# Arktis2022/Spiking-Diffusion

Measured on AMD Instinct MI355X. Metric: images/sec + LIF-kernel HBM GB/s, MNIST 100-step sample T=16, 1->8 GPU, higher is better.
Workload: dtype fp32-exact (4 fp6 digits x fp4 spikes on the block-scaled MFMA + certified decisions + exact 6-digit recomputation of flagged neurons)

## Files before the change

### spiking-diffusion_amd/csrc/cert_common.h

```cpp
#pragma once
#include "den_common.h"
#include <math.h>

typedef int v6i __attribute__((ext_vector_type(6)));
typedef int v8i __attribute__((ext_vector_type(8)));
typedef float v2f __attribute__((ext_vector_type(2)));
typedef float v16f __attribute__((ext_vector_type(16)));

constexpr int T16 = 16;
constexpr int POSB = 256;
constexpr int WT = 64 * 24;
constexpr float CERT_4EPS = 4.0f * 2.38418579e-07f;

constexpr unsigned FLAG_CAP = 1u << 20;
static inline long long spk_cert_bitmap_words(long long n) { return (n + 31) / 32; }
static inline long long spk_cert_ticket_idx(long long n) { return 2 + (long long)FLAG_CAP + spk_cert_bitmap_words(n); }
static inline long long spk_cert_flag_words(long long n) { return spk_cert_ticket_idx(n) + 1; }
struct CertWs { unsigned* flags; unsigned flag_cap; long long ticket_idx; };
static inline CertWs spk_cert_ws(unsigned* flag_words, int flag_cap, long long n) {
  return CertWs{flag_words, flag_cap < 0 || (unsigned)flag_cap > FLAG_CAP ? FLAG_CAP : (unsigned)flag_cap, spk_cert_ticket_idx(n)};
}

__device__ __forceinline__ unsigned* spk_cert_bitmap(const CertWs& ws) { return ws.flags + 2 + FLAG_CAP; }

__device__ __forceinline__ void spk_cert_flag(const CertWs& ws, long long n, bool flagged = true) {
  if (flagged) {
    const unsigned idx = atomicAdd(ws.flags, 1u);
    if (idx < ws.flag_cap) ws.flags[2 + idx] = (unsigned)n;
    else atomicOr(spk_cert_bitmap(ws) + (n >> 5), 1u << (n & 31));
  }
}

__device__ __forceinline__ void spk_cert_handover(const CertWs& ws) {
  if (atomicAdd(ws.flags + ws.ticket_idx, 1u) == gridDim.x - 1) {
    ws.flags[1] = atomicAdd(ws.flags, 0u);
    ws.flags[0] = 0u;
    ws.flags[ws.ticket_idx] = 0u;
  }
}

template <bool WG, class I, class Fix>
__device__ __forceinline__ void spk_cert_scan(const CertWs& ws, unsigned count, I unit, I n_units, long long n_words, bool clearer,
                                              Fix&& fix) {
  const unsigned nlist = count < ws.flag_cap ? count : ws.flag_cap;
  for (I e = unit; e < nlist; e += n_units) fix((long long)ws.flags[2 + e]);
  if (count > ws.flag_cap) {
    unsigned* bm = spk_cert_bitmap(ws);
    long long w0 = unit, w1 = n_words, step = n_units;
    if (WG) {
      const long long per = (n_words + n_units - 1) / n_units;
      w0 = (long long)unit * per;
      w1 = w0 + per < n_words ? w0 + per : n_words;
      step = 1;
    }
    for (long long wi = w0; wi < w1; wi += step) {
      unsigned wd = bm[wi];
      if (WG) __syncthreads();
      if (wd && clearer) bm[wi] = 0u;
      while (wd) {
        const int bit = __ffs((int)wd) - 1;
        wd &= wd - 1;
        fix(wi * 32 + bit);
      }
    }
  }
}

__device__ __forceinline__ void spk_cert_add_active8(long long& part, unsigned nib, const int4& q0, const int4& q1) {
  part += (nib & 0x0000000fu) ? (long long)q0.x : 0ll;
  part += (nib & 0x000000f0u) ? (long long)q0.y : 0ll;
  part += (nib & 0x00000f00u) ? (long long)q0.z : 0ll;
  part += (nib & 0x0000f000u) ? (long long)q0.w : 0ll;
  part += (nib & 0x000f0000u) ? (long long)q1.x : 0ll;
  part += (nib & 0x00f00000u) ? (long long)q1.y : 0ll;
  part += (nib & 0x0f000000u) ? (long long)q1.z : 0ll;
  part += (nib & 0xf0000000u) ? (long long)q1.w : 0ll;
}
__device__ __forceinline__ long long spk_join64(int lo, int hi) {
  return (long long)(((unsigned long long)(unsigned)hi << 32) | (unsigned)lo);
}
__device__ __forceinline__ long long spk_shfl64(long long v, int src) {
  return spk_join64(__shfl((int)(unsigned)(v & 0xffffffffll), src), __shfl((int)(v >> 32), src));
}
__device__ __forceinline__ long long spk_cert_sum_quarters(long long part) {
#pragma unroll
  for (int off = 16; off <= 32; off <<= 1)
    part += spk_join64(__shfl_xor((int)(unsigned)(part & 0xffffffffll), off), __shfl_xor((int)(part >> 32), off));
  return part;
}
__device__ __forceinline__ float exact_preact(double s, double sc, double bi) { return (float)fma(s, sc, bi); }
__device__ __forceinline__ void spk_cert_patch_nibble(uint8_t* rec, int co, bool spike) {
  const int byte = (co & 31) >> 1;
  unsigned* wp = reinterpret_cast<unsigned*>(rec + (byte & ~3));
  const unsigned shw = 8u * (byte & 3) + 4u * (co & 1);
  atomicAnd(wp, ~(0xFu << shw));
  if (spike) atomicOr(wp, 0x2u << shw);
}

__device__ __forceinline__ double spk_cert_quantise(float w, int sh) { return rint(ldexp((double)w, sh)); }
__device__ __forceinline__ void spk_cert_scale_bias(double* scale, double* bias_d, const float* bias, int co, int sh) {
  scale[co] = ldexp(1.0, -sh);
  bias_d[co] = bias ? (double)bias[co] : 0.0;
}
template <class Q>
__device__ __forceinline__ void spk_cert_emit_fragment(uint8_t* tile, int ln, int digit, bool live, Q&& q) {
  unsigned bits[6] = {0, 0, 0, 0, 0, 0};
  for (int k = 0; k < 32 && live; ++k) {
    int dg[6];
    spk_balanced_digits<5>(q(k), dg);
    int d = 0;
#pragma unroll
    for (int p = 0; p < 6; ++p) d = (p == digit) ? dg[p] : d;
    const unsigned code = spk_e2m3_code(d);
    const int bit = 6 * k, wd = bit >> 5, sft = bit & 31;
#pragma unroll
    for (int q2 = 0; q2 < 6; ++q2) {
      if (q2 == wd) bits[q2] |= code << sft;
      if (q2 == wd + 1 && sft > 26) bits[q2] |= code >> (32 - sft);
    }
  }
  unsigned* d16 = reinterpret_cast<unsigned*>(tile + ln * 16);
  unsigned* d8 = reinterpret_cast<unsigned*>(tile + 1024 + ln * 8);
  d16[0] = bits[0]; d16[1] = bits[1]; d16[2] = bits[2]; d16[3] = bits[3];
  d8[0] = bits[4]; d8[1] = bits[5];
}
```

### spiking-diffusion_amd/csrc/den_mfma_fp6v2.hip

```cpp
#include "cert_common.h"
#include "../../include/spkdiff.h"
#include <stdlib.h>
#include <type_traits>
#include <utility>

namespace {

constexpr int CK = 32;
constexpr int N_PAIR = 18;
constexpr int N_D4 = 5;
constexpr int N_MAIN = N_PAIR + N_D4;
constexpr int N_L5 = 2;
constexpr int NACC = 2;
constexpr int W_PIECES = (N_PAIR * WT + 1023) / 1024;
constexpr int W_LDS = W_PIECES * 1024;
constexpr int W_SLAB = ((N_MAIN + N_L5) * WT + 1023) / 1024 * 1024;

struct V2Args {
  const uint8_t* in0; int nch;
  const uint8_t* wq; const double* scale; const double* bias; const float* wl1;
  const float* bn_a; const float* bn_b;
  uint8_t* out; uint8_t* out_cnt;
  CertWs ws;
  int handover;
// ... 606 lines not shown
#pragma unroll
        for (int r = 0; r < 16; ++r) {
          const int rowA = spk_acc_row(r, 0);
          const int c0 = __builtin_amdgcn_readlane(cnt[i], rowA), c1 = __builtin_amdgcn_readlane(cnt[i], rowA + 4);
          cntv[r] = half ? c1 : c0;
        }
      }
      int nmax_rec = 0;
      if constexpr (REC) nmax_rec = s_nmax[BSKIP ? p_out[i] : 2 * (wave + NWV * i) + half];
      float zmax = 0.f, dmin = 3.0e38f;
      int nmax = nmax_rec;
#pragma unroll
      for (int r2 = 0; r2 < 16; r2 += 2) {
        const v2f p0 = {acc[i][0][r2], acc[i][0][r2 + 1]}, p1 = {acc[i][1][r2], acc[i][1][r2 + 1]};
        const v2f q4 = __builtin_elementwise_fma(p0, (v2f){1024.0f, 1024.0f}, p1);
        const v2f z2 = __builtin_elementwise_fma(q4, (v2f){Ac4, Ac4}, (v2f){Bc, Bc});
        if constexpr (!REC) nmax = max(nmax, max(cntv[r2], cntv[r2 + 1]));
#pragma unroll
        for (int e = 0; e < 2; ++e) {
          const float z = z2[e];
          zmax = fmaxf(zmax, fabsf(z));
          const float h = fmaf(z - v, 0.5f, v);
          const float hm = h - 1.0f;
          dmin = fminf(dmin, fabsf(hm));
          const bool s = h >= 1.0f;
          v = s ? 0.0f : h;
          mybits = __builtin_amdgcn_alignbit(mybits, __float_as_uint(hm), 31);
        }
      }
      mybits = ~(__builtin_bitreverse32(mybits) >> 16) & 0xffffu;
      flg = dmin <= SPK_V2_SPARE * fmaf(zmax, 2.5f * CERT_4EPS, fmaf((float)nmax, cT, cE));
      if (__builtin_amdgcn_ballot_w64(flg) != 0ull) {
        float v2 = 0.f, dh = 0.f;
        bool f2 = false;
        if constexpr (REC) {
          const v4i* rp = reinterpret_cast<const v4i*>(s_row + (BSKIP ? p_out[i] : 2 * (wave + NWV * i) + half) * 16);
#pragma unroll
          for (int q = 0; q < 4; ++q) {
            const v4i c4 = rp[q];
            cntv[4 * q] = c4[0]; cntv[4 * q + 1] = c4[1]; cntv[4 * q + 2] = c4[2]; cntv[4 * q + 3] = c4[3];
          }
        }
#pragma unroll
        for (int r2 = 0; r2 < 16; r2 += 2) {
          const v2f p0 = {acc[i][0][r2], acc[i][0][r2 + 1]}, p1 = {acc[i][1][r2], acc[i][1][r2 + 1]};
          const v2f q4 = __builtin_elementwise_fma(p0, (v2f){1024.0f, 1024.0f}, p1);
          const v2f z2 = __builtin_elementwise_fma(q4, (v2f){Ac4, Ac4}, (v2f){Bc, Bc});
#pragma unroll
          for (int e = 0; e < 2; ++e) {
            const float z = z2[e];
            const float ct = fmaf((float)cntv[r2 + e], cT, cE);
            dh = fmaf(fabsf(z) + fabsf(v2), 0.625f * CERT_4EPS, fmaf(dh, 0.5f, 0.5f * ct));
            const float h = fmaf(z - v2, 0.5f, v2);
            f2 = f2 || (fabsf(h - 1.0f) <= SPK_V2_SPARE * dh);
            v2 = h >= 1.0f ? 0.0f : h;
          }
        }
        flg = flg && f2;
      }
      const int ti = wave + NWV * i;
      const int p = (PRUNE || BSKIP) ? p_out[i] : 2 * ti + half + band * HWb;
      const bool listed = (!PRUNE || 2 * ti + half < n_list) && (!LIVE || b < n_live);
      if (flg && listed) spk_cert_flag(a.ws, ((long long)b * a.Cout + co) * HW + p);
      const long long rec = (((long long)b * G + g) * HW + p) * POSB;
      store_tile_spikes(a.out, a.out_cnt, mybits, lane, rec, (((long long)b * G + g) * HW + p) * 32, listed);
      __builtin_amdgcn_sched_barrier(0);
    }
  }
  spk_dma_wait_all();
}

__device__ __forceinline__ void fp6v2_wg_map(const V2Args& a, int& g, int& il, int& lanes) {
  const int k = blockIdx.x, G = a.Cout >> 5;
  if (a.gx > 0) {
    const int S = gridDim.x >> 3, x = k & 7, slot = k >> 3;
    const int npart = 8 / a.nsets, set = x % a.nsets, xi = x / a.nsets, lanes_x = S / a.gx;
    g = set * a.gx + slot % a.gx;
    il = xi * lanes_x + slot / a.gx;
    lanes = npart * lanes_x;
  } else {
    g = k % G;
    il = k / G;
    lanes = gridDim.x / G;
  }
}

__device__ __forceinline__ void fp6v2_handover(const V2Args& a) {
  if (!a.handover) return;
  __syncthreads();
  if (threadIdx.x == 0) spk_cert_handover(a.ws);
}

template <int H, int W, int NWV, bool SPLIT = false>
__global__ __launch_bounds__(NWV * 64, 1) void conv3x3_fp6v2_kernel(V2Args a) {
  const int Bn = spk_batch_count(a.n_dyn, a.B);
  int g, il, lanes;
  fp6v2_wg_map(a, g, il, lanes);
  if constexpr (NWV == 8 && !SPLIT) {
    switch (__builtin_amdgcn_readfirstlane((int)V2_WAVE_CLS[(threadIdx.x >> 6) & 7])) {
      case V2_TOP: fp6v2_body<H, W, NWV, false, 0, false, V2_TOP>(a, g, il, lanes, Bn, nullptr); break;
      case V2_RIGHT: fp6v2_body<H, W, NWV, false, 0, false, V2_RIGHT>(a, g, il, lanes, Bn, nullptr); break;
      case V2_LEFT: fp6v2_body<H, W, NWV, false, 0, false, V2_LEFT>(a, g, il, lanes, Bn, nullptr); break;
      case V2_BOTTOM: fp6v2_body<H, W, NWV, false, 0, false, V2_BOTTOM>(a, g, il, lanes, Bn, nullptr); break;
      default: fp6v2_body<H, W, NWV, false, 0, false, V2_INT>(a, g, il, lanes, Bn, nullptr); break;
    }
  } else fp6v2_body<H, W, NWV, SPLIT, 0>(a, g, il, lanes, Bn, nullptr);
  fp6v2_handover(a);
}

template <int H, int W>
__global__ __launch_bounds__(256, 1) void conv3x3_fp6v2_half_kernel(V2Args a) {
  const int Bn = spk_batch_count(a.n_dyn, a.B);
  int g, il, lanes;
  fp6v2_wg_map(a, g, il, lanes);
  fp6v2_body<H, W, 4, false, 3, true>(a, g, il, lanes, Bn, nullptr);
  fp6v2_handover(a);
}

template <int H, int W, int NWV>
__global__ __launch_bounds__(NWV * 64, 1) void conv3x3_fp6v2_listed_kernel(V2Args a) {
  constexpr int NC = (H * W / 2) / 4;
  const int Bn = spk_batch_count(a.n_dyn, a.B);
  int g, il, lanes;
  fp6v2_wg_map(a, g, il, lanes);
  int cnt[NC], work[NC], u[NC];
  int total = 0, nonempty = 0;
#pragma unroll
  for (int k = 0; k < NC; ++k) {
    cnt[k] = a.cls_cnt[k];
    work[k] = cnt[k] * (k + 1 < SPK_V2_KMIN ? SPK_V2_KMIN : k + 1);
    total += work[k];
    nonempty += cnt[k] > 0;
  }
  if (total == 0) { fp6v2_handover(a); return; }
  int rem = lanes - nonempty, used = 0;
#pragma unroll
  for (int k = 0; k < NC; ++k) {
    u[k] = cnt[k] > 0 ? 1 + (int)((long long)rem * work[k] / total) : 0;
    used += u[k];
  }
  for (int left = lanes - used; left > 0; --left) {
    int best = 0;
    long long bw = -1, bu = 1;
#pragma unroll
    for (int k = 0; k < NC; ++k)
      if (cnt[k] > 0 && (long long)work[k] * bu > bw * u[k]) { bw = work[k]; bu = u[k]; best = k; }
#pragma unroll
    for (int k = 0; k < NC; ++k) u[k] += (k == best);
  }
  int start = 0, cls = -1, il_c = 0, lanes_c = 1;
#pragma unroll
  for (int k = 0; k < NC; ++k) {
    if (il >= start && il < start + u[k]) { cls = k; il_c = il - start; lanes_c = u[k]; }
    start += u[k];
  }
  const int* slots = a.cls_list + (long long)(cls < 0 ? 0 : cls) * a.B;
  static_assert(NWV == 8, "listed positions: two waves per SIMD");
  switch (cls) {
    case 0: case 1: fp6v2_body<H, W, 8, false, 1>(a, g, il_c, lanes_c, cnt[cls], slots, Bn); break;
    case 2: case 3: fp6v2_body<H, W, 8, false, 2>(a, g, il_c, lanes_c, cnt[cls], slots, Bn); break;
    case 4: case 5: fp6v2_body<H, W, 8, false, 3>(a, g, il_c, lanes_c, cnt[cls], slots, Bn); break;
    default: break;
  }
  fp6v2_handover(a);
}


template <int H, int W, bool WIDE>
__device__ __forceinline__ void fp6v2_lastpos_body(const V2Args& a, const int bid, float (*red)[16][64]) {
  constexpr int HW = H * W, NP = SPK_V2_LP_PAIRS;
  const int lane = threadIdx.x & 63, wave = threadIdx.x >> 6;
  const int nch = a.nch, G = a.Cout >> 5;
  const int Bn = spk_batch_count(a.n_dyn, a.B);
  if (!a.handover && bid == 0 && threadIdx.x == 0) { a.ws.flags[1] = a.ws.flags[0]; a.ws.flags[0] = 0u; }
  const int n_units = ((Bn + 2 * NP - 1) / (2 * NP)) * G;
  const bool split = n_units <= SPK_V2_LP_SPLIT_MAX;
  const int unit = split ? bid : bid * 4 + wave;
  const int g = unit % G, b0 = (unit / G) * 2 * NP;
  if (b0 >= Bn) return;
  const int row = lane & 31, half = lane >> 5;
  const int hsel = (row >> 2) & 1, tt = (row & 3) + 4 * (row >> 3);
  const int sc_a = 0x7f7f7f7f;
  const int sc_p = half ? (int)0x82828282u : (int)0x87878787u;
  const int sc_hi = (int)0x87878787u, sc_lo = (int)0x82828282u;
  v16f acc[NP][3];
#pragma unroll
  for (int q = 0; q < NP; ++q)
#pragma unroll
    for (int j = 0; j < 3; ++j)
#pragma unroll
      for (int r = 0; r < 16; ++r) acc[q][j][r] = 0.f;
  const int py = H - 1, px = W - 1;
  for (int c = split ? wave : 0; c < nch; c += split ? 4 : 1) {
    const uint8_t* wslab = a.wq + ((long long)g * nch + c) * W_SLAB;
    auto ldb = [&](int tile) -> v8i {
      const uint8_t* wt = wslab + tile * WT;
      const v4i bx = *reinterpret_cast<const v4i*>(wt + lane * 16);
      const v2i by = *reinterpret_cast<const v2i*>(wt + 1024 + lane * 8);
      return v8i{bx[0], bx[1], bx[2], bx[3], by[0], by[1], 0, 0};
    };
    v4i sp[NP][4];
#pragma unroll
    for (int q = 0; q < NP; ++q) {
      const int bA = b0 + 2 * q + hsel;
#pragma unroll
      for (int u = 0; u < 4; ++u) {
        const int tap = (u >> 1) * 3 + (u & 1);
        const int yy = py + tap / 3 - 1, xx = px + tap % 3 - 1;
        sp[q][u] = v4i{0, 0, 0, 0};
        if (bA < Bn)
          sp[q][u] = *reinterpret_cast<const v4i*>(a.in0 + (((long long)bA * nch + c) * HW + yy * W + xx) * POSB + tt * 16);
      }
    }
    v8i bt[8];
#pragma unroll
    for (int u = 0; u < 4; ++u) {
      const int tap = (u >> 1) * 3 + (u & 1);
      bt[2 * u] = ldb(2 * tap); bt[2 * u + 1] = ldb(2 * tap + 1);
    }
    const v8i t18 = ldb(N_PAIR), t19 = ldb(N_PAIR + 1), t20 = ldb(N_PAIR + 2), t23 = ldb(N_MAIN), t24 = ldb(N_MAIN + 1);
    auto mm = [&](v16f& d, const v4i& av, const v8i& bv, int sb) {
      const v8i a8 = {av[0], av[1], av[2], av[3], 0, 0, 0, 0};
      d = __builtin_amdgcn_mfma_scale_f32_32x32x64_f8f6f4(a8, bv, d, 4, 2, 0, sc_a, 0, sb);
    };
    const v4i zero = {0, 0, 0, 0};
#pragma unroll
    for (int q = 0; q < NP; ++q) {
#pragma unroll
      for (int u = 0; u < 4; ++u) { mm(acc[q][0], sp[q][u], bt[2 * u], sc_p); mm(acc[q][1], sp[q][u], bt[2 * u + 1], sc_p); }
      const v4i a01 = half ? sp[q][1] : sp[q][0];
      const v4i az3 = half ? sp[q][2] : zero;
      const v4i a4z = half ? zero : sp[q][3];
      const v4i a34 = half ? sp[q][3] : sp[q][2];
      mm(acc[q][2], a01, t18, sc_hi); mm(acc[q][2], az3, t19, sc_hi); mm(acc[q][2], a4z, t20, sc_hi);
      mm(acc[q][2], a01, t23, sc_lo); mm(acc[q][2], a34, t24, sc_lo);
    }
  }
  if (split) {
    const int nw = nch < 4 ? nch : 4;
    if constexpr (WIDE) {
#pragma unroll
      for (int q = 0; q < NP; ++q) {
        if (q) __syncthreads();
        if (wave != 0 && wave < nw) {
#pragma unroll
          for (int j = 0; j < 3; ++j)
#pragma unroll
            for (int r = 0; r < 16; ++r) red[3 * (wave - 1) + j][r][lane] = acc[q][j][r];
        }
        __syncthreads();
        if (wave == 0) {
          for (int w = 1; w < nw; ++w)
#pragma unroll
            for (int j = 0; j < 3; ++j)
#pragma unroll
              for (int r = 0; r < 16; ++r) acc[q][j][r] += red[3 * (w - 1) + j][r][lane];
        }
      }
    } else {
#pragma unroll
      for (int q = 0; q < NP; ++q)
        for (int w = 1; w < 4; ++w) {
          if (wave == w && w < nw) {
#pragma unroll
            for (int j = 0; j < 3; ++j)
#pragma unroll
              for (int r = 0; r < 16; ++r) red[j][r][lane] = acc[q][j][r];
          }
          __syncthreads();
          if (wave == 0 && w < nw) {
#pragma unroll
            for (int j = 0; j < 3; ++j)
#pragma unroll
              for (int r = 0; r < 16; ++r) acc[q][j][r] += red[j][r][lane];
          }
          __syncthreads();
        }
    }
    if (wave != 0) return;
  }
  const int co = g * 32 + (lane & 31);
  const double sc = a.scale[co], bi = a.bias[co];
  const float bna = a.bn_a[co], bnb = a.bn_b[co];
#pragma unroll
  for (int q = 0; q < NP; ++q) {
    const int b = b0 + 2 * q + half;
    const bool ok = b < Bn;
    if (__builtin_amdgcn_ballot_w64(ok) == 0ull) continue;
    float v = 0.f;
    unsigned mybits = 0;
#pragma unroll
    for (int r = 0; r < 16; ++r) {
      const double s1 = fma((double)acc[q][0][r], 1024.0, (double)acc[q][1][r]);
      const double s = fma(s1, 1024.0, (double)acc[q][2][r]);
      const float y = exact_preact(s, sc, bi);
      const bool sp1 = spk_lif_step_default(v, fmaf(y, bna, bnb)) && ok;
      mybits |= sp1 ? (1u << r) : 0u;
    }
    const long long cell = ((long long)(ok ? b : 0) * G + g) * HW + (HW - 1);
    store_tile_spikes(a.out, a.out_cnt, mybits, lane, cell * POSB, cell * 32, ok);
  }
}

template <int H, int W>
__device__ __forceinline__ void fixup_neuron(const V2Args& a, long long n, unsigned long long* sS, int Bn) {
  constexpr int HW = H * W;
  const int tid = threadIdx.x, lane = tid & 63;
  const int nch = a.nch, Cin = a.Cin;
  const int p = (int)(n % HW);
  const long long r0 = n / HW;
  const int co = (int)(r0 % a.Cout), b = (int)(r0 / a.Cout);
  if (b >= Bn) return;
  const int py = p / W, px = p % W;
  if (tid < 16) sS[tid] = 0ull;
  long long part = 0;
  __syncthreads();
  const int units = 9 * nch * 16;
  for (int u = tid; u < units; u += (int)blockDim.x) {
    const int t = u & 15, cc = (u >> 4) % nch, tap = (u >> 4) / nch;
    const int yy = py + tap / 3 - 1, xx = px + tap % 3 - 1;
    if (yy < 0 || yy >= H || xx < 0 || xx >= W) continue;
    const uint4 sp = *reinterpret_cast<const uint4*>(a.in0 + (((long long)b * nch + cc) * HW + yy * W + xx) * POSB + t * 16);
    const int4* qp = reinterpret_cast<const int4*>(a.qtab + ((long long)co * 9 + tap) * Cin + cc * 32);
    const unsigned w4[4] = {sp.x, sp.y, sp.z, sp.w};
#pragma unroll
    for (int j = 0; j < 4; ++j) spk_cert_add_active8(part, w4[j], qp[2 * j], qp[2 * j + 1]);
  }
  part = spk_cert_sum_quarters(part);
  if (lane < 16 && part != 0) atomicAdd(&sS[lane], (unsigned long long)part);
  __syncthreads();
  if (tid < 64) {
    const double sc = a.scale[co], bi = a.bias[co];
    const float bna = a.bn_a[co], bnb = a.bn_b[co];
    float v = 0.f;
    unsigned bits = 0;
#pragma unroll
    for (int t = 0; t < 16; ++t) {
      const float y = exact_preact((double)(long long)sS[t], sc, bi);
      bits |= spk_lif_step_default(v, fmaf(y, bna, bnb)) ? (1u << t) : 0u;
    }
    const int g = co >> 5;
    if (lane < 16) {
      uint8_t* rec = a.out + ((((long long)b * (a.Cout >> 5) + g) * HW + p) * POSB);
      spk_cert_patch_nibble(rec + lane * 16, co, (bits >> lane) & 1u);
    }
    if (a.out_cnt && lane == 0) a.out_cnt[(((long long)b * (a.Cout >> 5) + g) * HW + p) * 32 + (co & 31)] = (uint8_t)__popc(bits);
  }
  __syncthreads();
}

template <int H, int W>
__device__ __forceinline__ void fp6v2_fixup_body(const V2Args& a, long long n_words, const unsigned bid, const unsigned nb,
                                                 unsigned long long* sS) {
  const int Bn = spk_batch_count(a.n_dyn, a.B);
  const unsigned count = a.ws.flags[a.handover ? 1 : 0];
  spk_cert_scan<true>(a.ws, count, bid, nb, n_words, threadIdx.x == 0,
                      [&](long long n) __attribute__((always_inline)) { fixup_neuron<H, W>(a, n, sS, Bn); });
}

constexpr int LPS_TILES = 13, LPS_BUF = LPS_TILES * WT;
constexpr int LPS_RING = 2;
constexpr size_t LPS_LDS = LPS_RING * (size_t)LPS_BUF;
static_assert(LPS_RING == 2 && 4 * (LPS_LDS + 128) <= 160 * 1024,
              "barrier c releases buffer (c + 1) % 2, the one chunk c - 1 was read from, never chunk c's; four workgroups per CU (128 B static each)");
template <int H, int W>
__device__ __forceinline__ void fp6v2_lastpos_shared_body(const V2Args& a, const int bid) {
  constexpr int HW = H * W;
  extern __shared__ __attribute__((aligned(16))) uint8_t lds[];
  const int lane = threadIdx.x & 63, wave = threadIdx.x >> 6;
  const int nch = a.nch, G = a.Cout >> 5;
  const int Bn = a.n_dyn ? (*a.n_dyn < a.B ? *a.n_dyn : a.B) : a.B;
  const int g = bid % G, b0 = (bid / G) * 8;
  if (b0 >= Bn) return;
  const int row = lane & 31, half = lane >> 5;
  const int hsel = (row >> 2) & 1, tt = (row & 3) + 4 * (row >> 3);
  const int sc_a = 0x7f7f7f7f;
  const int sc_p = half ? (int)0x82828282u : (int)0x87878787u;
  const int sc_hi = (int)0x87878787u, sc_lo = (int)0x82828282u;
  const int wave_s = __builtin_amdgcn_readfirstlane(wave);
  const unsigned lds_addr = spk_lds_addr(lds), lane16 = (unsigned)lane * 16u;
  auto issue_chunk = [&](int c, int buf) {
    const uint8_t* slab = a.wq + ((long long)g * nch + c) * W_SLAB;
#pragma unroll
    for (int k = 0; k < 5; ++k) {
      const int pc = 5 * wave_s + k;
      const int src = pc < 6 ? pc * 1024 : pc < 12 ? 6 * WT + (pc - 6) * 1024 : pc < 17 ? 18 * WT + (pc - 12) * 1024
                                                                                        : 23 * WT + (pc - 17) * 1024;
      const int dst = pc < 6 ? pc * 1024 : pc < 12 ? 4 * WT + (pc - 6) * 1024 : pc < 17 ? 8 * WT + (pc - 12) * 1024
                                                                                        : 11 * WT + (pc - 17) * 1024;
      const unsigned long long mask = pc == 16 ? 0xffffffffull : ~0ull;
      spk_dma16s_masked(slab + src, lane16, lds_addr + (unsigned)(buf * LPS_BUF + dst), mask);
    }
  };
  const int py = H - 1, px = W - 1;
  const int bA = b0 + 2 * wave + hsel, bAc = bA < Bn ? bA : Bn - 1;
  auto load_spikes = [&](int c, v4i (&sp)[4]) {
#pragma unroll
    for (int u = 0; u < 4; ++u) {
      const int tap = (u >> 1) * 3 + (u & 1);
      const int yy = py + tap / 3 - 1, xx = px + tap % 3 - 1;
      sp[u] = *reinterpret_cast<const v4i*>(a.in0 + (((long long)bAc * nch + c) * HW + yy * W + xx) * POSB + tt * 16);
    }
  };
  v16f acc[3];
#pragma unroll
  for (int j = 0; j < 3; ++j)
#pragma unroll
    for (int r = 0; r < 16; ++r) acc[j][r] = 0.f;
  v4i sp[4], spn[4];
  load_spikes(0, sp);
  issue_chunk(0, 0);
  asm volatile("" : "+v"(sp[0]), "+v"(sp[1]), "+v"(sp[2]), "+v"(sp[3]));
  for (int c = 0; c < nch; ++c) {
    const int buf = c & (LPS_RING - 1);
    asm volatile("s_waitcnt vmcnt(0)" ::: "memory");
    __syncthreads();
    load_spikes(c + 1 < nch ? c + 1 : c, spn);
    if (c + 1 < nch) issue_chunk(c + 1, buf ^ 1);
    const uint8_t* Wb = lds + buf * LPS_BUF;
    auto ldb = [&](int tile) -> v6i {
      const uint8_t* wt = Wb + tile * WT;
      const v4i bx = *reinterpret_cast<const v4i*>(wt + lane * 16);
      const v2i by = *reinterpret_cast<const v2i*>(wt + 1024 + lane * 8);
      return v6i{bx[0], bx[1], bx[2], bx[3], by[0], by[1]};
    };
    auto mm = [&](v16f& d, const v4i& av, const v6i& bv, int sb) { SPK_MFMA_FP6("v", d, av, bv, sc_a, sb); };
#pragma unroll
    for (int u = 0; u < 4; ++u) {
      const v6i t0 = ldb(2 * u), t1 = ldb(2 * u + 1);
      mm(acc[0], sp[u], t0, sc_p); mm(acc[1], sp[u], t1, sc_p);
      if (u & 1) __builtin_amdgcn_sched_barrier(0);
    }
    const v4i zero = {0, 0, 0, 0};
    const v4i a01 = half ? sp[1] : sp[0];
    const v4i az3 = half ? sp[2] : zero;
    const v4i a4z = half ? zero : sp[3];
    const v4i a34 = half ? sp[3] : sp[2];
    {
      const v6i t8 = ldb(8), t9 = ldb(9), t10 = ldb(10);
      mm(acc[2], a01, t8, sc_hi); mm(acc[2], az3, t9, sc_hi); mm(acc[2], a4z, t10, sc_hi);
    }
    __builtin_amdgcn_sched_barrier(0);
    {
      const v6i t11 = ldb(11), t12 = ldb(12);
      mm(acc[2], a01, t11, sc_lo); mm(acc[2], a34, t12, sc_lo);
    }
    __builtin_amdgcn_sched_barrier(0);
    asm volatile("" : "+v"(spn[0]), "+v"(spn[1]), "+v"(spn[2]), "+v"(spn[3]));
#pragma unroll
    for (int u = 0; u < 4; ++u) sp[u] = spn[u];
  }
  asm volatile("s_nop 15\n\ts_nop 15" ::: "memory");
  const int co = g * 32 + (lane & 31);
  const double sc = a.scale[co], bi = a.bias[co];
  const float bna = a.bn_a[co], bnb = a.bn_b[co];
  const int b = b0 + 2 * wave + half;
  const bool ok = b < Bn;
  if (__builtin_amdgcn_ballot_w64(ok) == 0ull) return;
  float v = 0.f;
  unsigned mybits = 0;
#pragma unroll
  for (int r = 0; r < 16; ++r) {
    const double s1 = fma((double)acc[0][r], 1024.0, (double)acc[1][r]);
    const double s2 = fma(s1, 1024.0, (double)acc[2][r]);
    const float y = exact_preact(s2, sc, bi);
    const bool sp1 = spk_lif_step_default(v, fmaf(y, bna, bnb)) && ok;
    mybits |= sp1 ? (1u << r) : 0u;
  }
  const long long cell = ((long long)(ok ? b : 0) * G + g) * HW + (HW - 1);
  store_tile_spikes(a.out, a.out_cnt, mybits, lane, cell * POSB, cell * 32, ok);
}

template <int H, int W, int PART>
__global__ __launch_bounds__(256, PART == 3 ? 4 : 1) void fp6v2_tail_kernel(V2Args a, long long n_words, int n_lp) {
  __shared__ float red[(PART == 1 || PART == 3) ? 1 : (PART == 2 ? 9 : 3)][16][64];
  __shared__ unsigned long long sS[16];
  if constexpr (PART == 3) {
    if ((int)blockIdx.x < n_lp) { if constexpr ((H * W) & 1) fp6v2_lastpos_shared_body<H, W>(a, (int)blockIdx.x); }
    else fp6v2_fixup_body<H, W>(a, n_words, blockIdx.x - (unsigned)n_lp, gridDim.x - (unsigned)n_lp, sS);
    (void)red;
  } else {
    if (PART == 2 || (PART == 0 && (int)blockIdx.x < n_lp)) fp6v2_lastpos_body<H, W, PART == 2>(a, (int)blockIdx.x, red);
    else fp6v2_fixup_body<H, W>(a, n_words, blockIdx.x - (unsigned)n_lp, gridDim.x - (unsigned)n_lp, sS);
  }
}

__global__ __launch_bounds__(256) void pack_fp6v2_kernel(const float* __restrict__ w, const float* __restrict__ bias,
                                                         uint8_t* __restrict__ wq, double* __restrict__ scale,
                                                         double* __restrict__ bias_d, float* __restrict__ wl1,
                                                         int* __restrict__ qtab, int Cout, int Cin) {
  __shared__ float smax[256];
  __shared__ double ssum[256];
  const int co = blockIdx.x, n = Cin * 9;
  const float* wc = w + (long long)co * n;
  float m = 0.f;
  for (int i = threadIdx.x; i < n; i += 256) m = fmaxf(m, fabsf(wc[i]));
  const int sh = 29 - spk_channel_exponent(smax, m);
  double l1 = 0.0;
  for (int i = threadIdx.x; i < n; i += 256) {
    const double q = spk_cert_quantise(wc[i], sh);
    l1 += fabs(q);
    const int ci = i / 9, tap = i - 9 * ci;
    qtab[((long long)co * 9 + tap) * Cin + ci] = (int)q;
  }
  ssum[threadIdx.x] = l1;
  __syncthreads();
  for (int s = 128; s > 0; s >>= 1) {
    if (threadIdx.x < s) ssum[threadIdx.x] += ssum[threadIdx.x + s];
    __syncthreads();
  }
  if (threadIdx.x == 0) {
    spk_cert_scale_bias(scale, bias_d, bias, co, sh);
    wl1[co] = (float)(ldexp(ssum[0], -sh) * 1.000001);
  }
  const int nchunks = Cin / CK, g = co >> 5, col = co & 31;
  constexpr int NTILE = N_MAIN + N_L5;
  for (int rec = threadIdx.x; rec < nchunks * NTILE * 2; rec += 256) {
    const int kh = rec & 1, tau = (rec >> 1) % NTILE, c = rec / (2 * NTILE);
    int tap, digit;
    bool valid = true;
    if (tau < N_PAIR) { tap = tau >> 1; digit = 2 * (tau & 1) + kh; }
    else if (tau < N_MAIN) { tap = 2 * (tau - N_PAIR) + kh; digit = 4; valid = tap < 9; }
    else { tap = (tau == N_MAIN ? 0 : 3) + kh; digit = 5; }
    spk_cert_emit_fragment(wq + (long long)(g * nchunks + c) * W_SLAB + tau * WT, kh * 32 + col, digit, valid,
                           [&](int j) { return (long long)spk_cert_quantise(wc[(c * CK + j) * 9 + tap], sh); });
  }
}

}

extern "C" long long spk_den_packed_weight_fp6v2_bytes(int Cout, int Cin) {
  if (Cout <= 0 || Cin <= 0 || (Cout % 32) || (Cin % CK)) return -1;
  return (long long)(Cout / 32) * (Cin / CK) * W_SLAB;
}

extern "C" int spk_den_pack_weight_fp6v2(const float* w, const float* bias, uint8_t* wq, double* scale, double* bias_d,
                                         float* wl1, int* qtab, int Cout, int Cin, hipStream_t stream) {
  if (!w || !wq || !scale || !bias_d || !wl1 || !qtab || Cout <= 0 || Cin <= 0) return SPK_ERR_ARG;
  if ((Cout % 32) || (Cin % CK)) return SPK_ERR_UNSUPPORTED;
  hipLaunchKernelGGL(pack_fp6v2_kernel, dim3(Cout), dim3(256), 0, stream, w, bias, wq, scale, bias_d, wl1, qtab, Cout, Cin);
  SPK_LAUNCH_CHECK();
  return SPK_OK;
}

extern "C" long long spk_den_fp6v2_flag_words(int B, int Cout, int H, int W) {
  if (B <= 0 || Cout <= 0 || H <= 0 || W <= 0) return -1;
  return spk_cert_flag_words((long long)B * Cout * H * W);
}

extern "C" int spk_den_conv3x3_mfma_fp6v2_supported(int Cout, int Cin, int k, int stride, int pad, int T, int H, int W) {
  return k == 3 && stride == 1 && pad == 1 && T == T16 && H == W && (H == 7 || H == 8) && Cout > 0 && Cin > 0 &&
         (Cout % 32) == 0 && (Cin % CK) == 0;
}

static int fp6v2_launch(const uint8_t* in_s32, int nch, const uint8_t* wq, const double* scale, const double* bias_d,
                        const float* wl1, const int* qtab, const float* bn_a, const float* bn_b, uint8_t* out_s32,
                        uint8_t* out_counts, unsigned* flag_words, int T, int B, int H, int W, int Cout,
                        const int* n_dyn_or_null, const uint8_t* need, int need_R, int need_r, int flag_cap, int form,
                        hipStream_t stream, int parts = 7) {
  const bool split_small = form == 0;
  if (!in_s32 || nch <= 0 || !wq || !scale || !bias_d || !wl1 || !qtab || !bn_a || !bn_b || !out_s32 || !flag_words ||
      B <= 0 || H <= 0 || W <= 0 || Cout <= 0)
    return SPK_ERR_ARG;
  if (!spk_den_conv3x3_mfma_fp6v2_supported(Cout, nch * CK, 3, 1, 1, T, H, W)) return SPK_ERR_UNSUPPORTED;
  const bool bands = H == 8;
  if (need && (bands || !n_dyn_or_null)) return SPK_ERR_UNSUPPORTED;
  V2Args a;
  a.in0 = in_s32; a.nch = nch; a.wq = wq; a.scale = scale; a.bias = bias_d; a.wl1 = wl1; a.qtab = qtab;
  a.bn_a = bn_a; a.bn_b = bn_b; a.out = out_s32; a.out_cnt = out_counts;
  a.ws = spk_cert_ws(flag_words, flag_cap, (long long)B * Cout * H * W);
  a.n_dyn = n_dyn_or_null;
  a.need = nullptr; a.cls_cnt = nullptr; a.cls_list = nullptr;
  if (need) {
    a.need = need + spk_need_off_rec(B, need_R, need_r);
    a.cls_cnt = reinterpret_cast<const int*>(need + spk_need_off_cnt(need_r));
    a.cls_list = reinterpret_cast<const int*>(need + spk_need_off_list(B, need_R, need_r));
  }
  a.B = B; a.Cout = Cout; a.Cin = nch * CK;
  const int cus = spk_cu_count();
  const int G = Cout / 32;
  int grid = 0;
  a.gx = 0; a.nsets = 1;
  const long long gx_kb = (n_dyn_or_null || need) ? 1536 : SPK_V2_GX_KB;
  auto xcd_walk = [&](V2Args& v, int wgs) -> int {
    v.gx = 0; v.nsets = 1;
    if ((wgs & 7) != 0) return 0;
    const int S = wgs / 8;
    int gx = 1;
    while (gx * 2 <= G && gx * 2 <= S && (long long)gx * 2 * nch * W_SLAB <= gx_kb * 1024) gx *= 2;
    while (G / gx > 8 && gx * 2 <= G && gx * 2 <= S) gx *= 2;
    const int nsets = G / gx;
    if (G % gx == 0 && nsets <= 8 && 8 % nsets == 0 && S % gx == 0) { v.gx = gx; v.nsets = nsets; return wgs; }
    return 0;
  };
  grid = xcd_walk(a, cus);
  if (a.gx == 0) grid = cus >= G ? (cus / G) * G : G;
  const int a_bytes = bands ? ((8 / 2 + 1 + 2) * 9 + 1) * POSB : ((7 + 2) * 8 + 1) * POSB;
  const size_t lds = 2 * ((size_t)a_bytes + W_LDS) + (size_t)((a_bytes / POSB) + (bands ? 32 : 49) + 1) * 64 + 256;
  const long long n_words = spk_cert_bitmap_words((long long)B * Cout * H * W);
  a.handover = 1;
  if (parts != 7) {
    if (parts == 2) {
      if (bands) hipLaunchKernelGGL((fp6v2_tail_kernel<8, 8, 1>), dim3(8 * cus), dim3(256), 0, stream, a, n_words, 0);
      else hipLaunchKernelGGL((fp6v2_tail_kernel<7, 7, 1>), dim3(8 * cus), dim3(256), 0, stream, a, n_words, 0);
    } else if (parts == 4 && !bands) {
      const int n_lp4 = ((B + 2 * SPK_V2_LP_PAIRS - 1) / (2 * SPK_V2_LP_PAIRS)) * G;
      hipLaunchKernelGGL((fp6v2_tail_kernel<7, 7, 2>), dim3(n_lp4), dim3(256), 0, stream, a, n_words, n_lp4);
    } else return SPK_ERR_UNSUPPORTED;
    SPK_LAUNCH_CHECK();
    return SPK_OK;
  }
  if (bands) {
    hipLaunchKernelGGL((conv3x3_fp6v2_kernel<8, 8, 8, true>), dim3(grid), dim3(512), lds, stream, a);
    SPK_LAUNCH_CHECK();
    hipLaunchKernelGGL((fp6v2_tail_kernel<8, 8, 1>), dim3(8 * cus), dim3(256), 0, stream, a, n_words, 0);
    SPK_LAUNCH_CHECK();
    return SPK_OK;
  }
  if (need) {
    if (grid / G < 6) return SPK_ERR_UNSUPPORTED;
    hipLaunchKernelGGL((conv3x3_fp6v2_listed_kernel<7, 7, 8>), dim3(grid), dim3(512), lds, stream, a);
  } else if (split_small && (long long)B * G * SPK_V2_HALF_FILL <= grid) {
    hipLaunchKernelGGL((conv3x3_fp6v2_half_kernel<7, 7>), dim3(grid), dim3(256), lds, stream, a);
  } else hipLaunchKernelGGL((conv3x3_fp6v2_kernel<7, 7, 8>), dim3(grid), dim3(512), lds, stream, a);
  SPK_LAUNCH_CHECK();
  const int n_lp = ((B + 2 * SPK_V2_LP_PAIRS - 1) / (2 * SPK_V2_LP_PAIRS)) * G;
  if (!n_dyn_or_null && nch >= 2 && B >= SPK_V2_LPS_MIN_B &&
      (long long)LPS_LDS + 4096 <= spk_lds_limit()) {
    const int n_lps = ((B + 7) / 8) * G;
    hipLaunchKernelGGL((fp6v2_tail_kernel<7, 7, 3>), dim3(n_lps + 4 * cus), dim3(256), LPS_LDS, stream, a, n_words, n_lps);
    SPK_LAUNCH_CHECK();
  } else {
    hipLaunchKernelGGL((fp6v2_tail_kernel<7, 7, 0>), dim3(n_lp + 8 * cus), dim3(256), 0, stream, a, n_words, n_lp);
    SPK_LAUNCH_CHECK();
  }
  return SPK_OK;
}

extern "C" int spk_den_conv3x3_mfma_fp6v2(const uint8_t* in_s32, int nch, const uint8_t* wq, const double* scale,
                                          const double* bias_d, const float* wl1, const int* qtab, const float* bn_a,
                                          const float* bn_b, uint8_t* out_s32, uint8_t* out_counts, unsigned* flag_words,
                                          int T, int B, int H, int W, int Cout, const int* n_dyn_or_null, int flag_cap,
                                          int form, hipStream_t stream) {
  if (form != 0 && form != 1) return SPK_ERR_ARG;
  return fp6v2_launch(in_s32, nch, wq, scale, bias_d, wl1, qtab, bn_a, bn_b, out_s32, out_counts, flag_words, T, B, H, W, Cout,
                      n_dyn_or_null, nullptr, 0, 0, flag_cap, form, stream);
}

extern "C" int spk_den_conv3x3_mfma_fp6v2_part(const uint8_t* in_s32, int nch, const uint8_t* wq, const double* scale,
                                               const double* bias_d, const float* wl1, const int* qtab, const float* bn_a,
                                               const float* bn_b, uint8_t* out_s32, uint8_t* out_counts, unsigned* flag_words,
                                               int T, int B, int H, int W, int Cout, const int* n_dyn_or_null, int part,
                                               int flag_cap, hipStream_t stream) {
  if (part != 2 && part != 4) return SPK_ERR_ARG;
  return fp6v2_launch(in_s32, nch, wq, scale, bias_d, wl1, qtab, bn_a, bn_b, out_s32, out_counts, flag_words, T, B, H, W, Cout,
                      n_dyn_or_null, nullptr, 0, 0, flag_cap, 1, stream, part);
}

extern "C" int spk_den_conv3x3_mfma_fp6v2_listed(const uint8_t* in_s32, int nch, const uint8_t* wq, const double* scale,
// ... 10 lines not shown
```

Before: 3356.

## Restructure certified fixup: row-per-unit loads, DPP weight broadcast, prefetched flag list

Rewrites the per-neuron exact recomputation so each 16-lane row handles one (tap, channel) unit. All spike and weight loads for up to nine trips are issued ahead of the accumulation. Each lane loads only two quantised weights and shares them across the row with DPP row broadcasts, where the old code had every lane read 32 weights. The flag-list scan now prefetches the next flagged neuron id while fixing the current one, and per-channel scale/bias loads are hoisted before the reduction. The aim is to cut memory traffic and latency in the fixup pass, at the cost of more registers and more complex indexing.

New measurement: 3380 (median of 6 runs). About the same (+0.7%).

```diff
diff --git a/spiking-diffusion_amd/csrc/cert_common.h b/spiking-diffusion_amd/csrc/cert_common.h
--- a/spiking-diffusion_amd/csrc/cert_common.h
+++ b/spiking-diffusion_amd/csrc/cert_common.h
@@ -40,10 +40,8 @@
 }
 
 template <bool WG, class I, class Fix>
-__device__ __forceinline__ void spk_cert_scan(const CertWs& ws, unsigned count, I unit, I n_units, long long n_words, bool clearer,
-                                              Fix&& fix) {
-  const unsigned nlist = count < ws.flag_cap ? count : ws.flag_cap;
-  for (I e = unit; e < nlist; e += n_units) fix((long long)ws.flags[2 + e]);
+__device__ __forceinline__ void spk_cert_scan_bitmap(const CertWs& ws, unsigned count, I unit, I n_units, long long n_words,
+                                                     bool clearer, Fix&& fix) {
   if (count > ws.flag_cap) {
     unsigned* bm = spk_cert_bitmap(ws);
     long long w0 = unit, w1 = n_words, step = n_units;
@@ -65,6 +63,28 @@
     }
   }
 }
+template <bool WG, class I, class Fix>
+__device__ __forceinline__ void spk_cert_scan(const CertWs& ws, unsigned count, I unit, I n_units, long long n_words, bool clearer,
+                                              Fix&& fix) {
+  const unsigned nlist = count < ws.flag_cap ? count : ws.flag_cap;
+  for (I e = unit; e < nlist; e += n_units) fix((long long)ws.flags[2 + e]);
+  spk_cert_scan_bitmap<WG>(ws, count, unit, n_units, n_words, clearer, fix);
+}
+template <class I, class Fix>
+__device__ __forceinline__ void spk_cert_scan_ahead(const CertWs& ws, const unsigned* count_at, I unit, I n_units, long long n_words,
+                                                    bool clearer, Fix&& fix) {
+  unsigned id = unit < FLAG_CAP ? ws.flags[2 + unit] : 0u;
+  const unsigned count = *count_at;
+  const unsigned nlist = count < ws.flag_cap ? count : ws.flag_cap;
+  for (I e = unit; e < nlist;) {
+    const I nx = e + n_units;
+    const unsigned id_nx = nx < FLAG_CAP ? ws.flags[2 + nx] : 0u;
+    fix((long long)id);
+    id = id_nx;
+    e = nx;
+  }
+  spk_cert_scan_bitmap<true>(ws, count, unit, n_units, n_words, clearer, fix);
+}
 
 __device__ __forceinline__ void spk_cert_add_active8(long long& part, unsigned nib, const int4& q0, const int4& q1) {
   part += (nib & 0x0000000fu) ? (long long)q0.x : 0ll;
@@ -75,6 +95,33 @@
   part += (nib & 0x00f00000u) ? (long long)q1.y : 0ll;
   part += (nib & 0x0f000000u) ? (long long)q1.z : 0ll;
   part += (nib & 0xf0000000u) ? (long long)q1.w : 0ll;
+}
+template <int L>
+__device__ __forceinline__ int spk_row_lane(int v) {
+  return __builtin_amdgcn_update_dpp(0, v, 0x150 + L, 0xf, 0xf, true);
+}
+__device__ __forceinline__ unsigned spk_nibbles_set(unsigned x) {
+  x |= x >> 1;
+  return x | (x >> 2);
+}
+template <int C>
+__device__ __forceinline__ int spk_cert_row_active(const unsigned (&set)[4], int wlo, int whi) {
+  if constexpr (C < 32) {
+    const int mask = (int)(set[C >> 3] << (31 - 4 * (C & 7))) >> 31;
+    return spk_row_lane<(C >> 1)>((C & 1) ? whi : wlo) & mask;
+  } else return 0;
+}
+template <int C = 0>
+__device__ __forceinline__ void spk_cert_add_row_from(long long& part, const unsigned (&set)[4], int wlo, int whi) {
+  if constexpr (C < 32) {
+    part += (long long)(spk_cert_row_active<C>(set, wlo, whi) + spk_cert_row_active<C + 1>(set, wlo, whi) +
+                        spk_cert_row_active<C + 2>(set, wlo, whi));
+    spk_cert_add_row_from<C + 3>(part, set, wlo, whi);
+  }
+}
+__device__ __forceinline__ void spk_cert_add_active32_row(long long& part, const uint4& sp, int wlo, int whi) {
+  const unsigned set[4] = {spk_nibbles_set(sp.x), spk_nibbles_set(sp.y), spk_nibbles_set(sp.z), spk_nibbles_set(sp.w)};
+  spk_cert_add_row_from(part, set, wlo, whi);
 }
 __device__ __forceinline__ long long spk_join64(int lo, int hi) {
   return (long long)(((unsigned long long)(unsigned)hi << 32) | (unsigned)lo);
diff --git a/spiking-diffusion_amd/csrc/den_mfma_fp6v2.hip b/spiking-diffusion_amd/csrc/den_mfma_fp6v2.hip
--- a/spiking-diffusion_amd/csrc/den_mfma_fp6v2.hip
+++ b/spiking-diffusion_amd/csrc/den_mfma_fp6v2.hip
@@ -932,36 +932,60 @@
   }
 }
 
+template <int H, int W, int K>
+__device__ __forceinline__ long long fixup_units(const V2Args& a, int b, int co, int py, int px, int first, int trips) {
+  constexpr int HW = H * W;
+  const int t = threadIdx.x & 15, row = (int)threadIdx.x >> 4;
+  const int nch = a.nch, Cin = a.Cin, q16 = 16 / nch, r16 = 16 % nch;
+  const uint8_t* in_b = a.in0 + (long long)b * nch * HW * POSB + t * 16;
+  const int* q_co = a.qtab + (long long)co * 9 * Cin + 2 * t;
+  long long part = 0;
+  uint4 sp[K];
+  int2 wq[K];
+  bool ok[K];
+  int tap = (first + row) / nch, cc = (first + row) % nch;
+#pragma unroll
+  for (int k = 0; k < K; ++k) {
+    ok[k] = false;
+    if (k < trips) {
+      const int yy = py + tap / 3 - 1, xx = px + tap % 3 - 1;
+      ok[k] = tap < 9 && yy >= 0 && yy < H && xx >= 0 && xx < W;
+      const int tapc = ok[k] ? tap : 4, cell = ok[k] ? yy * W + xx : py * W + px;
+      sp[k] = *reinterpret_cast<const uint4*>(in_b + ((long long)cc * HW + cell) * POSB);
+      wq[k] = *reinterpret_cast<const int2*>(q_co + tapc * Cin + cc * 32);
+      cc += r16; tap += q16;
+      if (cc >= nch) { cc -= nch; ++tap; }
+    }
+  }
+  __builtin_amdgcn_sched_barrier(0);
+#pragma unroll
+  for (int k = 0; k < K; ++k)
+    if (ok[k]) spk_cert_add_active32_row(part, sp[k], wq[k].x, wq[k].y);
+  return part;
+}
+
 template <int H, int W>
-__device__ __forceinline__ void fixup_neuron(const V2Args& a, long long n, unsigned long long* sS, int Bn) {
+__device__ __forceinline__ void fixup_neuron(const V2Args& a, long long n_any, unsigned long long* sS, int Bn) {
   constexpr int HW = H * W;
   const int tid = threadIdx.x, lane = tid & 63;
-  const int nch = a.nch, Cin = a.Cin;
+  const long long n = spk_join64(__builtin_amdgcn_readfirstlane((int)(unsigned)(n_any & 0xffffffffll)),
+                                 __builtin_amdgcn_readfirstlane((int)(n_any >> 32)));
   const int p = (int)(n % HW);
-  const long long r0 = n / HW;
-  const int co = (int)(r0 % a.Cout), b = (int)(r0 / a.Cout);
+  const unsigned r0 = (unsigned)(n / HW);
+  const int co = (int)(r0 % (unsigned)a.Cout), b = (int)(r0 / (unsigned)a.Cout);
   if (b >= Bn) return;
   const int py = p / W, px = p % W;
+  const double sc = a.scale[co], bi = a.bias[co];
+  const float bna = a.bn_a[co], bnb = a.bn_b[co];
   if (tid < 16) sS[tid] = 0ull;
-  long long part = 0;
+  const int trips = (9 * a.nch + 15) >> 4;
+  long long part = fixup_units<H, W, 9>(a, b, co, py, px, 0, trips);
+  for (int first = 16 * 9; first < 9 * a.nch; first += 16) part += fixup_units<H, W, 1>(a, b, co, py, px, first, 1);
   __syncthreads();
-  const int units = 9 * nch * 16;
-  for (int u = tid; u < units; u += (int)blockDim.x) {
-    const int t = u & 15, cc = (u >> 4) % nch, tap = (u >> 4) / nch;
-    const int yy = py + tap / 3 - 1, xx = px + tap % 3 - 1;
-    if (yy < 0 || yy >= H || xx < 0 || xx >= W) continue;
-    const uint4 sp = *reinterpret_cast<const uint4*>(a.in0 + (((long long)b * nch + cc) * HW + yy * W + xx) * POSB + t * 16);
-    const int4* qp = reinterpret_cast<const int4*>(a.qtab + ((long long)co * 9 + tap) * Cin + cc * 32);
-    const unsigned w4[4] = {sp.x, sp.y, sp.z, sp.w};
-#pragma unroll
-    for (int j = 0; j < 4; ++j) spk_cert_add_active8(part, w4[j], qp[2 * j], qp[2 * j + 1]);
-  }
   part = spk_cert_sum_quarters(part);
   if (lane < 16 && part != 0) atomicAdd(&sS[lane], (unsigned long long)part);
   __syncthreads();
   if (tid < 64) {
-    const double sc = a.scale[co], bi = a.bias[co];
-    const float bna = a.bn_a[co], bnb = a.bn_b[co];
     float v = 0.f;
     unsigned bits = 0;
 #pragma unroll
@@ -983,8 +1007,7 @@
 __device__ __forceinline__ void fp6v2_fixup_body(const V2Args& a, long long n_words, const unsigned bid, const unsigned nb,
                                                  unsigned long long* sS) {
   const int Bn = spk_batch_count(a.n_dyn, a.B);
-  const unsigned count = a.ws.flags[a.handover ? 1 : 0];
-  spk_cert_scan<true>(a.ws, count, bid, nb, n_words, threadIdx.x == 0,
+  spk_cert_scan_ahead(a.ws, a.ws.flags + (a.handover ? 1 : 0), bid, nb, n_words, threadIdx.x == 0,
                       [&](long long n) __attribute__((always_inline)) { fixup_neuron<H, W>(a, n, sS, Bn); });
 }
 
```
